# coezmaden/GPUAcceleratedTracking

Hardware: AMD Instinct MI355X
Metric: Msamples/s downconvert+correlate (E/P/L x ants x sats); real-time factor @ 1ms (higher is better)
Workload: dtype f32

## Files before the change

gpuacceleratedtracking_amd/csrc/gat_api.cpp:

```cpp
#include <algorithm>
#include <cctype>
#include <cmath>
#include <cstdio>
#include <cstdlib>
#include <cstring>
#include <ctime>
#include <dlfcn.h>
#include <new>
#include <string>
#include <vector>

#include "gat_ctx.h"

using namespace gat;

namespace gat {

struct Roctx {
    int (*push)(const char *) = nullptr;
    int (*pop)() = nullptr;
    Roctx()
    {
        const char *e = std::getenv("GAT_ROCTX");
        if (e && e[0] == '0') return;
// ... 133 lines not shown
            }
            c->loop_graphs.erase(c->loop_graphs.begin() + (long)lru);
        }
        gat_ctx::LoopGraph g;
        g.key = key;
        g.exec = exec;
        g.last_use = ++c->loop_graph_clock;
        c->loop_graphs.push_back(std::move(g));
    }
    if (graph) (void)hipGraphDestroy(graph);
    return GAT_OK;
}

void key_put_ctx(std::vector<unsigned char> &key, const gat_ctx *c)
{
    key_put(key, c->mc_mode); key_put(key, c->mc_i16_terms); key_put(key, c->mc_nct); key_put(key, c->max_aw); key_put(key, c->max_kt); key_put(key, c->max_bpw); key_put(key, c->force_bpw);
    key_put(key, c->wgs_per_cu); key_put(key, c->max_depth); key_put(key, c->one_wave); key_put(key, c->keep_l2); key_put(key, c->align_head);
    key_put(key, c->aw2); key_put(key, c->quads); key_put(key, c->bit_tables); key_put(key, c->seg_cap);
    key_put(key, c->d_codes); key_put(key, c->d_code_bits); key_put(key, c->Lc); key_put(key, c->P);
    key_put(key, c->d_partial); key_put(key, c->partial_bytes);
}

}

namespace {

struct OptionDesc {
    const char *name;
    long long lo, hi;
};
constexpr OptionDesc kOptions[] = {
// ... 3 lines not shown
    {"dc_kt", 1, 4},
    {"dc_bpw", 1, 1 << 20},
    {"dc_bpw_force", 0, 1 << 20},
    {"dc_wgs_per_cu", 0, 1024},
    {"dc_one_wave", 0, 1},
    {"dc_one_wave_min", -1, 1ll << 40},
    {"dc_ow_seg", 1, kUcarSteps},
    {"dc_depth", 1, 2},
    {"dc_keep_l2", -1, 1},
    {"dc_quads", -1, 1},
    {"dc_bits", 0, 2},
    {"dc_aw2", -1, 1},
    {"dc_seg", 0, kUcarSteps},
    {"mc_nct", 0, 4},
    {"mc_i16_terms", 2, 3},
    {"dc_align", 0, 1},
};

int32_t set_option(gat_ctx *c, const char *name, long long v)
{
    const OptionDesc *o = nullptr;
    for (const auto &d : kOptions)
        if (std::strcmp(d.name, name) == 0) o = &d;
    if (!o) return fail(c, GAT_ERR_ARG, "unknown option");
    if (v < o->lo || v > o->hi) return fail(c, GAT_ERR_RANGE, "option value out of range");
    const std::string n = name;
    if (n == "sync_flag_wgs") c->flag_max_wgs = (int)v;
    else if (n == "max_ant_tile") c->max_ant_tile = (int)v;
    else if (n == "dc_aw") c->max_aw = (int)v;
    else if (n == "dc_kt") c->max_kt = (int)v;
    else if (n == "dc_bpw") c->max_bpw = (int)v;
    else if (n == "dc_bpw_force") c->force_bpw = (int)v;
    else if (n == "dc_wgs_per_cu") c->wgs_per_cu = (int)v;
    else if (n == "dc_one_wave") c->one_wave = (int)v;
    else if (n == "dc_one_wave_min") c->one_wave_min = v;
    else if (n == "dc_ow_seg") c->one_wave_seg = (int)v;
    else if (n == "dc_depth") c->max_depth = (int)v;
    else if (n == "dc_keep_l2") c->keep_l2 = (int)v;
    else if (n == "dc_quads") c->quads = (int)v;
    else if (n == "dc_bits") c->bit_tables = (int)v;
    else if (n == "dc_aw2") c->aw2 = (int)v;
    else if (n == "dc_seg") c->seg_cap = (int)v;
    else if (n == "dc_align") c->align_head = (int)v;
    else if (n == "mc_i16_terms") c->mc_i16_terms = (int)v;
    else if (n == "mc_nct") c->mc_nct = v == 3 ? 2 : (int)v;
    return GAT_OK;
}

}

extern "C" {

GAT_API int32_t gat_create(int32_t device, void *hip_stream, gat_ctx **out_ctx)
{
    if (!out_ctx) return GAT_ERR_ARG;
    *out_ctx = nullptr;
    int ndev = 0;
    hipError_t e = hipGetDeviceCount(&ndev);
    if (e != hipSuccess) return -(int32_t)e;
// ... 621 lines not shown
```

gpuacceleratedtracking_amd/csrc/gat_ctx.h:

```cpp
#pragma once

#include <cmath>
#include <string>
#include <vector>

#include "gat_internal.h"

struct gat_ctx;

struct gat_resident {
    gat_ctx *ctx = nullptr;
    hipStream_t stream = nullptr;
    gat::DcArgs a{};
    gat::DcLaunch cfg{};
    gat::ResidentArgs r{};
    unsigned char *h_block = nullptr;
    unsigned *h_bell = nullptr, *h_state = nullptr, *h_lines = nullptr, *h_init = nullptr;
    unsigned *d_quit = nullptr;
    unsigned *d_bell = nullptr;
    int bell_copies = 1;
    int wgs = 0, lines_per_wg = 0, nval = 0;
    int blocks_per_cu = 1;
    std::vector<int> val_src, val_dst;
    unsigned seq = 0;
// ... 49 lines not shown
    int force_bpw = 0;
    int wgs_per_cu = 0;
    int one_wave = 1;
    long long one_wave_min = -1;
    int one_wave_seg = gat::kOneWaveSegSteps;
    int max_depth = 2;
    int keep_l2 = -1;
    int quads = -1;
    int bit_tables = 1;
    int aw2 = -1;
    int seg_cap = 0;
    int align_head = 1;
    int mc_mode = 1;
    int mc_nct = 0;
    int mc_i16_terms = 2;
    std::string err;
    gat_launch_info last{};
};

namespace gat {

inline int32_t fail(gat_ctx *c, int32_t code, const char *msg)
{
    if (c) c->err = msg;
    return code;
}

inline int32_t hipfail(gat_ctx *c, hipError_t e, const char *where)
{
    if (c) {
// ... 45 lines not shown
```

gpuacceleratedtracking_amd/csrc/gat_internal.h:

```cpp
#pragma once

#include <hip/hip_runtime.h>
#include <stdint.h>

#include "gat.h"

#if (defined(GAT_DC_ABLATE) || defined(GAT_DC_LAT_CUT) || defined(GAT_ABLATE) || defined(GAT_MFMA_STAMPS) || defined(GAT_MB_CW8) || defined(GAT_MB_NT_LOADS) || defined(GAT_MB_NO_RING) || defined(GAT_MB_X2_ITEMS4) || defined(GAT_MB_X2_DEPTH2) || \
     defined(GAT_RES_STAMPS) || defined(GAT_RES_FENCE)) &&                                                                                                 \
    !defined(GAT_DEV)
#error "diagnostic builds (-DGAT_DC_ABLATE, -DGAT_DC_LAT_CUT, -DGAT_ABLATE, -DGAT_MFMA_STAMPS, -DGAT_MB_CW8, -DGAT_RES_STAMPS, -DGAT_RES_FENCE) need -DGAT_DEV"
#endif

namespace gat {

constexpr int kThreads = 256;
constexpr int kMaxTapsPerLaunch = 8;
constexpr int kInlineParams = 4;
constexpr int kMaxAntTile = 4;
constexpr int kFinalizeFewSplits = 32;
constexpr int kMaxReplicaSpan = 512;
constexpr int kMaxLaunchSpan = 2048;

#ifndef GAT_PLANAR_GROUPS
#define GAT_PLANAR_GROUPS 1
// ... 205 lines not shown
constexpr int mb_consumer_waves(int, int) { return 4; }
#endif
constexpr int kMbMaxChain = 8192;
constexpr int kMbMaxSlots = 24;
constexpr int kMbHeader = 1536;
constexpr int mb_tile_samples(int RT, int NCT)
{
    const int t = 32 * (4 / NCT), cap = 128 / RT;
    return t < cap ? t : cap;
}
constexpr int mb_slots(int nct, int L, int K)
{
    const int s = (32 * nct + 2 * L - 1) / (2 * L) + 1;
    return s < K ? s : K;
}
enum MbMode : int { kMbThree = 0, kMbOne = 1, kMbTwo = 2 };
constexpr int mb_mode(int rt, int nct, int fmt, bool force_three = false)
{
    if (fmt == GAT_LAYOUT_INTERLEAVED_I8) return kMbOne;
    const int wpt = mb_consumer_waves(rt, nct) / nct, hs = mb_tile_samples(rt, nct) / (wpt > 0 ? wpt : 1) / 2;
    return fmt == GAT_LAYOUT_INTERLEAVED_I16 && !force_three && wpt > 0 && hs >= 8 && hs % 8 == 0 ? kMbTwo : kMbThree;
}
constexpr int mb_two_row_bytes(int T) { return ((10 * T + 15) / 16 * 16) | 16; }
#ifdef GAT_MB_NO_RING
constexpr bool mb_rep_ring_rows(int) { return false; }
#else
constexpr bool mb_rep_ring_rows(int rt) { return rt >= 2; }
#endif
constexpr int mb_rep_ring(int rt, int T, int span) { return mb_rep_ring_rows(rt) ? (span + 2 * T + T - 1) / T * T : 0; }
constexpr int mb_rep_row(int rt, int T, int span) { return mb_rep_ring_rows(rt) ? mb_rep_ring(rt, T, span) + span + T : span + T; }
constexpr size_t mb_lds_bytes(int rt, int nct, int fmt, int nslots, int rep_stride, int code_bits_stride, int mode = -1)
{
    if (mode < 0) mode = mb_mode(rt, nct, fmt);
    const bool x1 = mode == kMbOne;
    const int T = mb_tile_samples(rt, nct);
    const int xs = x1 ? T + 2 : T + 1, wbytes = x1 ? 8 : 16;
    const size_t xw = mode == kMbTwo ? (size_t)2 * rt * 32 * mb_two_row_bytes(T) + (size_t)2 * (2 * nslots + 1) * mb_two_row_bytes(T)
                                     : (size_t)2 * rt * 32 * xs * 8 + (size_t)2 * (2 * nslots + 1) * xs * wbytes;
    return (size_t)kMbHeader + xw + (size_t)(((mb_rep_ring_rows(rt) ? 1 : 2) * nslots * rep_stride + 3) & ~3) * 4 + (size_t)nslots * code_bits_stride * 4;
}
constexpr int kMfTile = 256;
constexpr int kMfXStride = kMfTile + 1;
constexpr size_t mf_lds_bytes(int nct, int ct, int rep_stride, int code_row_stride, int codes_in_lds)
{
    return (size_t)1024 + (size_t)2 * 32 * kMfXStride * sizeof(float) + (size_t)2 * nct * ct * rep_stride * sizeof(float) +
           (codes_in_lds ? (size_t)nct * ct * code_row_stride + 16 : 0);
}
hipError_t launch_mfma(const MfArgs &a, int nct, unsigned grid, unsigned lds_bytes, hipStream_t s);
size_t mfma_lds_bytes(int nct, int ct, int rep_stride, int code_row_stride, int codes_in_lds);
hipError_t launch_mfma_bf16(const MfArgs &a, int rt, int nct, int fmt, unsigned grid, unsigned lds_bytes, hipStream_t s);
size_t mfma_bf16_lds_bytes(int rt, int nct, int fmt, int nslots, int rep_stride, int code_bits_stride, int mode);
int mfma_bf16_mode(int rt, int nct, int fmt, bool force_three);
// ... 40 lines not shown
```

gpuacceleratedtracking_amd/csrc/gat_mfma_bf16.hip:

```cpp
#include "gat_internal.h"
#include "gat_phase.h"

#include <utility>

namespace gat {

typedef float f32x16 __attribute__((ext_vector_type(16)));
typedef float f32x4_ __attribute__((ext_vector_type(4)));
typedef short bf16x8 __attribute__((ext_vector_type(8)));
typedef unsigned u32x4 __attribute__((ext_vector_type(4)));
typedef unsigned u32x2 __attribute__((ext_vector_type(2)));

namespace {

constexpr int consumer_waves(int RT, int NCT) { return mb_consumer_waves(RT, NCT); }
constexpr int kMaxChain = kMbMaxChain;
constexpr int kReanchor = 16;
constexpr int kHeader = kMbHeader;

struct Split3 {
    unsigned v, r, r2;
};
__device__ __forceinline__ Split3 split3(float v)
{
    Split3 s;
    s.v = __float_as_uint(v);
    const float r = v - __uint_as_float(s.v & 0xffff0000u);
    s.r = __float_as_uint(r);
    s.r2 = __float_as_uint(r - __uint_as_float(s.r & 0xffff0000u));
    return s;
}
__device__ __forceinline__ void gload_nt(f32x4_ &dst, const void *p)
{
#ifdef GAT_MB_NT_LOADS
    asm volatile("global_load_dwordx4 %0, %1, off nt" : "=v"(dst) : "v"(p) : "memory");
#else
    asm volatile("global_load_dwordx4 %0, %1, off" : "=v"(dst) : "v"(p) : "memory");
#endif
}
template <int XI>
__device__ __forceinline__ void wait_loads(f32x4_ (&xv)[XI])
{
    static_assert(XI >= 1 && XI <= 4, "prefetch group size");
    if constexpr (XI == 1)
// ... 13 lines not shown
    u32x4 w;
    unsigned m;
    u32x2 xa[RT];
#if defined(GAT_ABLATE) && (GAT_ABLATE & 64)
    u32x2 wl;
#endif
};
template <int RT>
struct FragSet<RT, kMbOne> {
    u32x4 w;
    u32x2 m;
    u32x4 xa[RT];
#if defined(GAT_ABLATE) && (GAT_ABLATE & 64)
    u32x2 wl;
#endif
};
template <int RT>
struct FragSet<RT, kMbTwo> {
    u32x4 w;
    u32x2 m;
    unsigned m3;
    u32x4 xa[RT];
};
template <int RT, int XM>
constexpr int frag_reads(int J) { return XM == kMbTwo ? 2 + RT + ((J % 5 == 1 || J % 5 == 3) ? 1 : 0) : 2 + RT; }
template <int RT, int XM>
constexpr int frag_newer(int J, int n, int NM)
{
    int c = 0;
    for (int i = 1; i <= n; ++i) c += frag_reads<RT, XM>((J + i) % NM);
// ... 11 lines not shown
    }
#endif
#if defined(GAT_ABLATE) && (GAT_ABLATE & 64)
    asm volatile("ds_read_b64 %0, %1 offset:%2" : "=v"(s.wl) : "v"(w_addr), "n"(J * 16));
#else
    asm volatile("ds_read_b128 %0, %1 offset:%2" : "=v"(s.w) : "v"(w_addr), "n"(J * 16));
#endif
    if constexpr (XM == kMbTwo) {
        constexpr int j = J % 5, sb = 8 * (J / 5);
        constexpr int o0 = sb + (j == 0 ? 0 : j == 1 ? 1 : j == 2 ? 3 : j == 3 ? 4 : 6);
        asm volatile("ds_read2_b32 %0, %1 offset0:%2 offset1:%3" : "=v"(s.m) : "v"(r_addr), "n"(o0), "n"(o0 + 1));
        if constexpr (j == 1 || j == 3) asm volatile("ds_read_b32 %0, %1 offset:%2" : "=v"(s.m3) : "v"(r_addr), "n"((o0 + 2) * 4));
#pragma unroll
        for (int t = 0; t < RT; ++t)
            asm volatile("ds_read_b128 %0, %1 offset:%2" : "=v"(s.xa[t]) : "v"(x_addr[t]), "n"(J * 16));
    } else if constexpr (XM == kMbOne) {
        asm volatile("ds_read2_b32 %0, %1 offset0:%2 offset1:%3" : "=v"(s.m) : "v"(r_addr), "n"(2 * J), "n"(2 * J + 1));
#pragma unroll
        for (int t = 0; t < RT; ++t)
            asm volatile("ds_read_b128 %0, %1 offset:%2" : "=v"(s.xa[t]) : "v"(x_addr[t]), "n"(J * 16));
    } else {
        asm volatile("ds_read_b32 %0, %1 offset:%2" : "=v"(s.m) : "v"(r_addr), "n"(J * 4));
#pragma unroll
        for (int t = 0; t < RT; ++t)
            asm volatile("ds_read_b64 %0, %1 offset:%2" : "=v"(s.xa[t]) : "v"(x_addr[t]), "n"(J * 8));
    }
}
template <int RT, int XM, int NEWER>
__device__ __forceinline__ void frag_wait(FragSet<RT, XM> &s)
{
// ... 10 lines not shown
                         : "n"(NEWER));
    } else if constexpr (RT == 1)
        asm volatile("s_waitcnt lgkmcnt(%3)" : "+v"(s.w), "+v"(s.m), "+v"(s.xa[0]) : "n"(NEWER));
    else if constexpr (RT == 2)
        asm volatile("s_waitcnt lgkmcnt(%4)" : "+v"(s.w), "+v"(s.m), "+v"(s.xa[0]), "+v"(s.xa[1]) : "n"(NEWER));
    else
        asm volatile("s_waitcnt lgkmcnt(%6)"
                     : "+v"(s.w), "+v"(s.m), "+v"(s.xa[0]), "+v"(s.xa[1]), "+v"(s.xa[2]), "+v"(s.xa[3])
                     : "n"(NEWER));
}
template <int RT, int XM = kMbThree>
constexpr int frag_depth()
{
    constexpr int per = XM == kMbTwo ? 3 + RT : 2 + RT;
#ifndef GAT_MB_X2_DEPTH2
    if ((XM == kMbTwo || XM == kMbOne) && RT == 4) return 1;
#endif
    return (15 / per) < 4 ? (15 / per) : 4;
}

template <int RT, int XM>
using FragRing = FragSet<RT, XM>[frag_depth<RT, XM>() + 1];

template <int J, int RT, int XM>
__device__ __forceinline__ void mfma_apply(f32x16 (&acc)[RT == 1 ? 2 : RT], FragSet<RT, XM> &cur);

template <int J, int NM, int RT, int XM>
__device__ __forceinline__ void mfma_slice(f32x16 (&acc)[RT == 1 ? 2 : RT], FragRing<RT, XM> &fs, unsigned w_addr,
                                           unsigned r_addr, const unsigned (&x_addr)[RT])
{
    constexpr int D = frag_depth<RT, XM>();
// ... 26 lines not shown
#endif
    if constexpr (XM == kMbTwo) {
        const unsigned A = cur.m[0], B = cur.m[1], C = cur.m3;
        constexpr int j = J % 5;
        auto LH = [](unsigned a_, unsigned b_) { return GAT_PERM(b_, a_, 0x07060100u); };
        if constexpr (j == 0) { w[0] ^= A; w[1] ^= A; w[2] ^= LH(A, B); w[3] ^= B; }
        else if constexpr (j == 1) { w[0] ^= A; w[1] ^= B; w[2] ^= B; w[3] ^= LH(B, C); }
        else if constexpr (j == 2) { w[0] ^= A; w[1] ^= A; w[2] ^= B; w[3] ^= B; }
        else if constexpr (j == 3) { w[0] ^= LH(A, B); w[1] ^= B; w[2] ^= B; w[3] ^= C; }
        else { w[0] ^= A; w[1] ^= LH(A, B); w[2] ^= B; w[3] ^= B; }
        const bf16x8 bw = __builtin_bit_cast(bf16x8, w);
#pragma unroll
        for (int t = 0; t < RT; ++t)
            acc[RT == 1 ? (J & 1) : t] = __builtin_amdgcn_mfma_f32_32x32x16_bf16(__builtin_bit_cast(bf16x8, cur.xa[t]), bw,
                                                                             acc[RT == 1 ? (J & 1) : t], 0, 0, 0);
    } else if constexpr (X1) {
        const unsigned m0 = cur.m[0], m1 = cur.m[1];
        w[0] ^= m0;
        w[1] ^= m0;
        w[2] ^= m1;
        w[3] ^= m1;
        const bf16x8 bw = __builtin_bit_cast(bf16x8, w);
#pragma unroll
        for (int t = 0; t < RT; ++t)
            acc[RT == 1 ? (J & 1) : t] = __builtin_amdgcn_mfma_f32_32x32x16_bf16(__builtin_bit_cast(bf16x8, cur.xa[t]), bw,
                                                                             acc[RT == 1 ? (J & 1) : t], 0, 0, 0);
    } else {
        const unsigned mk = cur.m;
        w[0] ^= mk;
        w[1] ^= mk;
// ... 70 lines not shown
    float wTr, wTi;
    int prn, valid, bad;
    int inc_ok;
};
static_assert(sizeof(ChanInfoB) == 64, "ChanInfoB layout");

constexpr int tile_samples(int RT, int NCT) { return mb_tile_samples(RT, NCT); }

}

template <int RT, int NCT, int FMT, int XM>
__global__ void __launch_bounds__(mb_threads(RT, NCT)) mfma_bf16_kernel(const MfArgs a)
{
    static_assert((XM == kMbOne) == (FMT == GAT_LAYOUT_INTERLEAVED_I8), "one term: int8 samples, and only they");
    static_assert(XM != kMbTwo || FMT == GAT_LAYOUT_INTERLEAVED_I16, "two terms: int16 samples");
    constexpr int kMbThreads = mb_threads(RT, NCT);
    constexpr int T = tile_samples(RT, NCT);
    constexpr int NCW = consumer_waves(RT, NCT);
    constexpr int WPT = NCW / NCT;
    constexpr int SW = T / WPT;
    constexpr bool X1 = XM == kMbOne;
    constexpr bool X2 = XM == kMbTwo;
    constexpr int SPS = X1 ? 4 : 2;
    constexpr int NM = X2 ? 5 * (SW / 2) / 8 : SW / SPS;
    static_assert(!X2 || (SW / 2) % 8 == 0, "two-term stream: 8 samples per half and period");
    constexpr int OS = XM == kMbThree ? T / 2 : 1;
#ifdef GAT_MB_X2_ITEMS4
    constexpr int IS = X2 ? 4 : 2;
#else
    constexpr int IS = 2;
#endif
    constexpr int RB = mb_two_row_bytes(T);
    constexpr int XS = X1 ? T + 2 : T + 1;
    constexpr int WS = X1 ? T + 2 : T + 1;
    constexpr int WE = X1 ? 1 : 2;
    constexpr bool PLANAR = FMT == GAT_LAYOUT_PLANAR;
    constexpr int GS = PLANAR ? 4 : FMT == GAT_LAYOUT_INTERLEAVED ? 2 : FMT == GAT_LAYOUT_INTERLEAVED_I16 ? 4 : 8;
    constexpr int BYTES = FMT == GAT_LAYOUT_INTERLEAVED_I16 ? 4 : FMT == GAT_LAYOUT_INTERLEAVED_I8 ? 2 : 8;
    constexpr int QPR = T / GS;
    constexpr int PT = kMbThreads - 64 * NCW;
    constexpr int NG = (PLANAR ? RT * 32 : RT * 16) * QPR;
    extern __shared__ __attribute__((aligned(16))) unsigned char smem[];
    const int L = a.L;
    const int nslots = a.nslots;
    const int wrows = 2 * nslots + 1;
    const int RS = a.rep_stride;
    ChanInfoB *s_chan = reinterpret_cast<ChanInfoB *>(smem);
    u32x2 *s_x = reinterpret_cast<u32x2 *>(smem + kHeader);
    u32x2 *s_w = X2 ? s_x + 2 * RT * 32 * (RB / 8) : s_x + 2 * RT * 32 * XS;
    constexpr bool RINGREP = mb_rep_ring_rows(RT);
    unsigned *s_rep = reinterpret_cast<unsigned *>(X2 ? s_w + 2 * wrows * (RB / 8) : s_w + 2 * wrows * WS * WE);
    unsigned *s_code = s_rep + (((RINGREP ? 1 : 2) * nslots * RS + 3) & ~3);
    const int RR = a.rep_ring, WIN = a.rep_span + tile_samples(RT, NCT);
    auto ring_next = [RR](int s_) {
        const int n = s_ + tile_samples(RT, NCT), m = (n - RR) >> 31;
        return (n & m) | ((n - RR) & ~m);
    };

    const int tid = threadIdx.x, lane = tid & 63, wave = tid >> 6;
    const bool producer = wave >= NCW;
    const int ptid = tid - 64 * NCW;

    const unsigned xcd = blockIdx.x & 7u, jq = blockIdx.x >> 3;
    const int cg = (int)(jq % (unsigned)a.chan_groups);
    unsigned tile = (jq / (unsigned)a.chan_groups) * 8u + xcd;
    if (tile >= (unsigned)a.num_tiles) return;
// ... 19 lines not shown
            ci.phi = P.carrier_phase_cycles;
            const double sp = __builtin_fabs(ci.tau) + __builtin_fabs(ci.ratio) * (double)(N + a.max_abs_shift) + 1.0;
            ci.bad = P.prn < 0 || P.prn >= a.num_prns || !(sp < 1073741824.0) || !(sp < 2097152.0 * (double)Lc) ||
                     !(ci.ratio >= 0.0) || !(ci.ratio * 32.0 < (double)Lc) || carrier_bad(ci.step, ci.phi);
            ci.prn = (P.prn < 0 || P.prn >= a.num_prns) ? 0 : P.prn;
            if (ci.bad) { ci.ratio = 0.0; ci.tau = 0.0; ci.step = 0.0; ci.phi = 0.0; }
            carrier_reduce(ci.step, ci.phi);
            const double st_O = ci.step * (double)OS;
            sincos_cycles(st_O - __builtin_rint(st_O), ci.wr, ci.wi);
            const double st_T = ci.step * (double)T;
            sincos_cycles(st_T - __builtin_rint(st_T), ci.wTr, ci.wTi);
            ci.inc_ok = ci.ratio * (double)(T + 2) < (double)Lc;
        }
        s_chan[tid] = ci;
    }
    if constexpr (X2) {
        for (int e = tid; e < 2 * (RB / 8); e += kMbThreads)
            s_w[((e / (RB / 8)) * wrows + 2 * nslots) * (RB / 8) + e % (RB / 8)] = u32x2{0u, 0u};
    } else {
        for (int e = tid; e < 2 * WS * WE; e += kMbThreads)
            s_w[((e / (WS * WE)) * wrows * WS + 2 * nslots * WS) * WE + e % (WS * WE)] = u32x2{0u, 0u};
    }
    __syncthreads();
    {
        const int vec_per_row = a.code_bits_stride / 4;
        for (int e = tid; e < nslots * vec_per_row; e += kMbThreads) {
            const int slot = e / vec_per_row, v = e - slot * vec_per_row;
            const ChanInfoB c = s_chan[slot];
            if (c.valid)
                reinterpret_cast<uint4 *>(s_code)[slot * vec_per_row + v] =
                    reinterpret_cast<const uint4 *>(a.code_bits + (size_t)c.prn * a.code_bits_stride)[v];
// ... 68 lines not shown
                    u32x2 *d = reinterpret_cast<u32x2 *>(reinterpret_cast<unsigned char *>(xb) + plane * RB + 40 * q);
                    d[0] = u32x2{GAT_P2(A[0], A[0]), GAT_P2(B[0], A[0])};
                    d[1] = u32x2{GAT_P2(A[1], B[0]), GAT_P2(A[1], A[1])};
                    d[2] = u32x2{GAT_P2(B[1], B[1]), GAT_P2(A[2], A[2])};
                    d[3] = u32x2{GAT_P2(B[2], A[2]), GAT_P2(A[3], B[2])};
                    d[4] = u32x2{GAT_P2(A[3], A[3]), GAT_P2(B[3], B[3])};
                };
                put4(2 * row, ar, br);
                put4(2 * row + 1, ai, bi);
                continue;
            }
            auto put = [&](int plane, int rel, float v) {
                if constexpr (X1) {
                    const unsigned fb = __float_as_uint(v);
                    xb[plane * XS + rel] = u32x2{GAT_PERM(fb, fb, 0x03020302u), fb >> 16};
                } else {
#if defined(GAT_ABLATE) && (GAT_ABLATE & 128)
                    const unsigned fb = __float_as_uint(v);
                    const float r = v - __uint_as_float(fb & 0xffff0000u);
                    xb[plane * XS + rel] = u32x2{GAT_PERM(__float_as_uint(r), fb, 0x07060302u), 0u};
#else
                    const Split3 sp = split3(v);
                    xb[plane * XS + rel] = u32x2{GAT_PERM(sp.r, sp.v, 0x07060302u), GAT_PERM(sp.r2, sp.r2, 0x03020302u)};
#endif
                }
            };
            if constexpr (PLANAR) {
#pragma unroll
                for (int u = 0; u < 4; ++u) put(row, 4 * q + u, xv[it][u]);
            } else if constexpr (FMT == GAT_LAYOUT_INTERLEAVED) {
// ... 47 lines not shown
                row[e] = m;
                return;
            }
            int q = win + e;
            q -= q >= RR ? RR : 0;
            row[q] = m;
            if (q < WIN) row[RR + q] = m;
        };
        put(e0, m0);
        if (e0 + dist < e_end) put(e0 + dist, m1);
    };
    float car_r = 0.f, car_i = 0.f;
    int rep_ip = 0, rep_t = 0, rep_ip2 = 0, rep_t2 = 0;
    const int item_i = ptid / (T / IS), item_q = ptid % (T / IS);
    const int item_slot = X2 ? ((item_i & ~3) | ((item_i & 1) << 1) | ((item_i >> 1) & 1)) : item_i;
    const int item_s0 = X2 ? IS * item_q : X1 ? 2 * item_q : item_q;
    const bool have_item = producer && item_slot < nslots;
    int p_win = 0;
    auto produce = [&](int st, int buf, bool first) {
        const int nb = st * T;
        const int win = p_win;
        if constexpr (RINGREP) p_win = ring_next(p_win);
        u32x2 *wb = X2 ? s_w + buf * wrows * (RB / 8) : s_w + buf * wrows * WS * WE;
        unsigned *rb = RINGREP ? s_rep : s_rep + buf * nslots * RS;
        const ChanInfoB c = s_chan[have_item ? item_slot : 0];
        if (first) {
            const int gps = (span + 1) >> 1;
            for (int id = ptid; id < nslots * gps; id += PT) {
                const int slot = id / gps, g = id - slot * gps;
                const ChanInfoB cs = s_chan[slot];
                if (!cs.valid) continue;
                int ip_unused, t_unused;
                gen_rep2(cs, s_code + slot * a.code_bits_stride, rb + slot * RS, win, nb, 2 * g, 1, span, true, ip_unused, t_unused);
            }
        } else if constexpr (!RINGREP) {
            const unsigned *rprev = s_rep + (buf ^ 1) * nslots * RS;
            const int pw = wave - NCW;
            for (int slot = pw; slot < nslots; slot += PT / 64)
// ... 13 lines not shown
                         anchor || !c.inc_ok, rep_ip2, rep_t2);
        }
#if defined(GAT_ABLATE) && (GAT_ABLATE & 2)
        if (!first) return;
#endif
        float cr, ci;
        if (anchor) {
            const double th = __builtin_fma((double)(nb + item_s0), c.step, c.phi);
            sincos_cycles(th - __builtin_rint(th), cr, ci);
        } else {
            cr = __builtin_fmaf(car_r, c.wTr, -(car_i * c.wTi));
            ci = __builtin_fmaf(car_r, c.wTi, car_i * c.wTr);
        }
        car_r = cr;
        car_i = ci;
        if constexpr (X2 && IS == 2) {
            const Split3 c0 = split3(cr), s0 = split3(-ci);
            const float tr = __builtin_fmaf(cr, c.wr, -(ci * c.wi));
            ci = __builtin_fmaf(cr, c.wi, ci * c.wr);
            cr = tr;
            const Split3 c1 = split3(cr), s1 = split3(-ci);
            unsigned *dre = reinterpret_cast<unsigned *>(reinterpret_cast<unsigned char *>(wb) + (2 * item_slot) * RB + 20 * item_q);
            unsigned *dim = reinterpret_cast<unsigned *>(reinterpret_cast<unsigned char *>(dre) + RB);
            dre[0] = GAT_P2(c0.r, c0.v); dre[1] = GAT_P2(c0.v, c0.r2); dre[2] = GAT_P2(c1.v, c0.r); dre[3] = GAT_P2(c1.r2, c1.r); dre[4] = GAT_P2(c1.r, c1.v);
            dim[0] = GAT_P2(s0.r, s0.v); dim[1] = GAT_P2(s0.v, s0.r2); dim[2] = GAT_P2(s1.v, s0.r); dim[3] = GAT_P2(s1.r2, s1.r); dim[4] = GAT_P2(s1.r, s1.v);
            return;
        } else if constexpr (X2) {
            unsigned ch[4], cm[4], cl[4], sh[4], sm[4], sl[4];
#pragma unroll
            for (int u = 0; u < 4; ++u) {
                const Split3 sc = split3(cr), ss = split3(-ci);
// ... 41 lines not shown
        }
    };

    const int cw = producer ? 0 : wave;
    const int ctl = cw / WPT;
    const int sub = cw % WPT;
    const int r = lane & 31, h = lane >> 5;
    const int col = 32 * (NCT * cg + ctl) + r;
    const int k_col = col / (2 * L), rem_col = col - 2 * L * k_col;
    const int l = rem_col >> 1, comp = rem_col & 1;
    const bool in_range = k_col < a.K && k_col - k_first < nslots;
    const int slot_c = in_range ? k_col - k_first : 0;
    const ChanInfoB my = s_chan[slot_c];
    const bool live_col = in_range && my.valid;
    const int col0 = sub * SW + h * (SW / 2);
    const int w_off = X2 ? (live_col ? 2 * slot_c + comp : 2 * nslots) * RB + 10 * col0 : (live_col ? 2 * slot_c + comp : 2 * nslots) * WS + col0;
    const int r_off = slot_c * RS + (a.shifts[l] - a.shifts[0]) + col0;
    const int x_off = X2 ? r * RB + 10 * col0 : r * XS + col0;
    constexpr int XBUF = X2 ? RT * 32 * RB : 8 * RT * 32 * XS, XTILE = X2 ? 32 * RB : 8 * 32 * XS, XU = X2 ? 1 : 8;
    const int WBUF = X2 ? wrows * RB : 8 * WE * wrows * WS, WU = X2 ? 1 : 8 * WE;

    if (!producer) __builtin_amdgcn_s_setprio(3);

    constexpr int NA = RT == 1 ? 2 : RT;
    f32x16 acc[NA];
#pragma unroll
    for (int t = 0; t < NA; ++t)
#pragma unroll
        for (int i = 0; i < 16; ++i) acc[t][i] = 0.f;

    const unsigned lds_x = (unsigned)(uintptr_t)s_x, lds_w = (unsigned)(uintptr_t)s_w, lds_r = (unsigned)(uintptr_t)s_rep;
    int c_win = 0;
    auto consume = [&](int buf) {
#if defined(GAT_ABLATE) && (GAT_ABLATE & 8)
        return;
// ... 212 lines not shown

int mfma_bf16_slots(int nct, int L, int K) { return mb_slots(nct, L, K); }

size_t mfma_bf16_lds_bytes(int rt, int nct, int fmt, int nslots, int rep_stride, int code_bits_stride, int mode)
{
    static_assert(sizeof(ChanInfoB) * kMbMaxSlots <= kHeader, "channel table must fit the header");
    return mb_lds_bytes(rt, nct, fmt, nslots, rep_stride, code_bits_stride, mode);
}
int mfma_bf16_mode(int rt, int nct, int fmt, bool force_three) { return mb_mode(rt, nct, fmt, force_three); }

namespace {
template <int RT, int NCT, int F>
hipError_t launch_one(const MfArgs &a, dim3 g, dim3 blk, unsigned lds_bytes, hipStream_t s)
{
    constexpr int natural = F == GAT_LAYOUT_INTERLEAVED_I8 ? kMbOne : kMbThree;
    if constexpr (mb_mode(RT, NCT, F) == kMbTwo) {
        if (a.mb_mode == kMbTwo) {
            hipLaunchKernelGGL((mfma_bf16_kernel<RT, NCT, F, kMbTwo>), g, blk, lds_bytes, s, a);
            return hipSuccess;
        }
    }
    if (a.mb_mode != natural) return hipErrorInvalidValue;
    hipLaunchKernelGGL((mfma_bf16_kernel<RT, NCT, F, natural>), g, blk, lds_bytes, s, a);
    return hipSuccess;
}
}

hipError_t launch_mfma_bf16(const MfArgs &a, int rt, int nct, int fmt, unsigned grid, unsigned lds_bytes, hipStream_t s)
{
    const dim3 g(grid), blk(mb_threads(rt, nct));
// ... 20 lines not shown
```

gpuacceleratedtracking_amd/csrc/gat_planner.cpp:

```cpp
#include <algorithm>
#include <cctype>
#include <cmath>
#include <cstdio>
#include <cstdlib>
#include <cstring>
#include <ctime>
#include <dlfcn.h>
#include <new>
#include <string>
#include <vector>

#include "gat_ctx.h"

using namespace gat;

int32_t gat::correlate_impl(gat_ctx *c, const gat_signal_desc *sig, const gat_channel_params *params_dev,
                            int32_t B, int32_t K, int32_t L, const int32_t *shifts, double fs,
                            float *out_re, float *out_im, uint32_t flags, const gat_channel_params *params_inline,
                            DcPlan *plan_out)
{
    c->wait_seq = 0;
    const TraceRange trace("gat_downconvert_and_correlate");
    if (!sig || (!params_dev && !params_inline) || !shifts || !out_re || !out_im) return fail(c, GAT_ERR_ARG, "null argument");
    if (!c->d_codes) return fail(c, GAT_ERR_STATE, "gat_set_codes has not been called");
// ... 90 lines not shown
        const bool round2_rule = M >= 32 && K >= 32 && (long long)M * K >= 2048;
        const bool auto_bf16 = 2ll * L * K >= 24 && (int8_in || (L <= 3 ? util >= util_min : round2_rule));
        const bool auto_f32 = false;
        const bool want_bf16 = c->mc_mode == 3 || (c->mc_mode == 1 && auto_bf16);
        const bool want_f32 = c->mc_mode == 2 || (c->mc_mode == 1 && auto_f32);
        int kind = 0, rt = 1, rep_stride_m = 0;
        int nslots_b = 0, nct_b = 1;
        if (shape_any && want_bf16 && c->d_code_bits && c->d_zeros && N % spv == 0 && spv <= 8) {
            if (c->mc_nct > 0) n_first = c->mc_nct;
            for (int n = n_first; n >= 1 && !kind; n >>= 1) {
                rt = (rt_max == 4 && n == 1) ? 2 : rt_max;
                const int T = mfma_bf16_tile_samples(rt, n);
                int rs = ((mb_rep_row(rt, T, (int)span) + 31) / 32) * 32 + 1;
                const int ns = mfma_bf16_slots(n, L, K);
                if (ns * T / 2 > mfma_bf16_producer_threads(rt, n) || ns > mfma_bf16_max_slots()) continue;
                const int mode_n = mfma_bf16_mode(rt, n, fmt, c->mc_i16_terms == 3);
                const int rs_tuned = pick_rep_stride(rs - 1, tiles_b, order);
                if (mfma_bf16_lds_bytes(rt, n, fmt, ns, rs_tuned, c->code_bits_stride, mode_n) <= 160 * 1024) rs = rs_tuned;
                if (mfma_bf16_lds_bytes(rt, n, fmt, ns, rs, c->code_bits_stride, mode_n) <= 160 * 1024) {
                    if (c->mc_mode == 1) {
                        const long long steps_total = (N + T - 1) / T;
                        const long long groups = (long long)B * (M / (16 * rt)) * ((tiles_b + n - 1) / n);
                        const long long cut = std::min<long long>(steps_total, std::max<long long>(1, (2ll * c->num_cus + groups - 1) / groups));
                        const long long steps_each = (steps_total + cut - 1) / cut;
                        if (steps_each < (two_term || int8_in ? 16 : 32)) break;
                    }
                    kind = 2;
                    nct_b = n;
                    nslots_b = ns;
                    rep_stride_m = rs;
                }
// ... 76 lines not shown
            m.partial = c->d_partial;
#ifdef GAT_MFMA_STAMPS
            {
                static unsigned long long *dbg = nullptr;
                if (!dbg) hipMalloc(reinterpret_cast<void **>(&dbg), 8u << 20);
                m.dbg = dbg;
                c->dbg_ptr = dbg;
            }
#endif
            unsigned lds;
            if (kind == 2) {
                m.codes_in_lds = 1;
                m.code_bits = c->d_code_bits;
                m.zeros = c->d_zeros;
                m.code_bits_stride = c->code_bits_stride;
                m.mb_mode = mfma_bf16_mode(rt, nct, fmt, c->mc_i16_terms == 3);
                lds = (unsigned)mfma_bf16_lds_bytes(rt, nct, fmt, m.nslots, m.rep_stride, c->code_bits_stride, m.mb_mode);
                GAT_HIP(c, launch_mfma_bf16(m, rt, nct, fmt, (unsigned)grid_m, lds, c->stream));
            } else {
                m.codes_in_lds = mfma_lds_bytes(nct, CT, m.rep_stride, c->code_row_stride, 1) <= 160 * 1024;
                lds = (unsigned)mfma_lds_bytes(nct, CT, m.rep_stride, c->code_row_stride, m.codes_in_lds);
                GAT_HIP(c, launch_mfma(m, nct, (unsigned)grid_m, lds, c->stream));
            }
            const bool fin_m = !atomic_m && m.splits > 1;
            if (fin_m)
                GAT_HIP(c, launch_finalize(c->d_partial, out_re, out_im, m.splits, L * M * 2, (long long)B * K, c->stream));
            c->last.workgroups = (int32_t)grid_m;
            c->last.threads = kind == 2 ? mfma_bf16_threads(rt, nct) : 2 * kThreads;
            c->last.splits = m.splits;
            c->last.ant_tile = kind == 2 ? 16 * rt : 16;
            c->last.vec = 4;
// ... 274 lines not shown
```

Measured before the change: 214,500.

## Add six-product bf16 split mode for float samples in MFMA correlator

Adds a kMbSix mode for f32 planar/interleaved samples. Each sample and carrier value is split into three RNE bf16 terms, and only six of the nine cross products are fed to the MFMA, replacing the previous three-term path. It packs the carrier terms into 12-byte-per-sample rows and reads them with ds_read2/ds_read_b128 patterns. The aim is to cut MFMA and LDS work per sample while keeping near-f32 accuracy, at the risk of slight precision loss and extra producer split work. It is on by default (mc_f32_products=6) and can be turned off via an option.

```diff
diff --git a/gpuacceleratedtracking_amd/csrc/gat_api.cpp b/gpuacceleratedtracking_amd/csrc/gat_api.cpp
--- a/gpuacceleratedtracking_amd/csrc/gat_api.cpp
+++ b/gpuacceleratedtracking_amd/csrc/gat_api.cpp
@@ -171,7 +171,7 @@
 
 void key_put_ctx(std::vector<unsigned char> &key, const gat_ctx *c)
 {
-    key_put(key, c->mc_mode); key_put(key, c->mc_i16_terms); key_put(key, c->mc_nct); key_put(key, c->max_aw); key_put(key, c->max_kt); key_put(key, c->max_bpw); key_put(key, c->force_bpw);
+    key_put(key, c->mc_mode); key_put(key, c->mc_i16_terms); key_put(key, c->mc_f32_products); key_put(key, c->mc_nct); key_put(key, c->max_aw); key_put(key, c->max_kt); key_put(key, c->max_bpw); key_put(key, c->force_bpw);
     key_put(key, c->wgs_per_cu); key_put(key, c->max_depth); key_put(key, c->one_wave); key_put(key, c->keep_l2); key_put(key, c->align_head);
     key_put(key, c->aw2); key_put(key, c->quads); key_put(key, c->bit_tables); key_put(key, c->seg_cap);
     key_put(key, c->d_codes); key_put(key, c->d_code_bits); key_put(key, c->Lc); key_put(key, c->P);
@@ -205,6 +205,7 @@
     {"dc_seg", 0, kUcarSteps},
     {"mc_nct", 0, 4},
     {"mc_i16_terms", 2, 3},
+    {"mc_f32_products", 6, 8},
     {"dc_align", 0, 1},
 };
 
@@ -215,6 +216,7 @@
         if (std::strcmp(d.name, name) == 0) o = &d;
     if (!o) return fail(c, GAT_ERR_ARG, "unknown option");
     if (v < o->lo || v > o->hi) return fail(c, GAT_ERR_RANGE, "option value out of range");
+    if (std::strcmp(name, "mc_f32_products") == 0 && v == 7) return fail(c, GAT_ERR_RANGE, "option value out of range");
     const std::string n = name;
     if (n == "sync_flag_wgs") c->flag_max_wgs = (int)v;
     else if (n == "max_ant_tile") c->max_ant_tile = (int)v;
@@ -234,6 +236,7 @@
     else if (n == "dc_seg") c->seg_cap = (int)v;
     else if (n == "dc_align") c->align_head = (int)v;
     else if (n == "mc_i16_terms") c->mc_i16_terms = (int)v;
+    else if (n == "mc_f32_products") c->mc_f32_products = (int)v;
     else if (n == "mc_nct") c->mc_nct = v == 3 ? 2 : (int)v;
     return GAT_OK;
 }
diff --git a/gpuacceleratedtracking_amd/csrc/gat_ctx.h b/gpuacceleratedtracking_amd/csrc/gat_ctx.h
--- a/gpuacceleratedtracking_amd/csrc/gat_ctx.h
+++ b/gpuacceleratedtracking_amd/csrc/gat_ctx.h
@@ -87,6 +87,7 @@
     int mc_mode = 1;
     int mc_nct = 0;
     int mc_i16_terms = 2;
+    int mc_f32_products = 6;
     std::string err;
     gat_launch_info last{};
 };
diff --git a/gpuacceleratedtracking_amd/csrc/gat_internal.h b/gpuacceleratedtracking_amd/csrc/gat_internal.h
--- a/gpuacceleratedtracking_amd/csrc/gat_internal.h
+++ b/gpuacceleratedtracking_amd/csrc/gat_internal.h
@@ -243,14 +243,17 @@
     const int s = (32 * nct + 2 * L - 1) / (2 * L) + 1;
     return s < K ? s : K;
 }
-enum MbMode : int { kMbThree = 0, kMbOne = 1, kMbTwo = 2 };
-constexpr int mb_mode(int rt, int nct, int fmt, bool force_three = false)
+enum MbMode : int { kMbThree = 0, kMbOne = 1, kMbTwo = 2, kMbSix = 3 };
+constexpr int mb_mode(int rt, int nct, int fmt, bool force_three = false, int f32_products = 6)
 {
     if (fmt == GAT_LAYOUT_INTERLEAVED_I8) return kMbOne;
     const int wpt = mb_consumer_waves(rt, nct) / nct, hs = mb_tile_samples(rt, nct) / (wpt > 0 ? wpt : 1) / 2;
+    if (fmt == GAT_LAYOUT_PLANAR || fmt == GAT_LAYOUT_INTERLEAVED)
+        return f32_products == 6 && wpt > 0 && hs >= 4 && hs % 4 == 0 ? kMbSix : kMbThree;
     return fmt == GAT_LAYOUT_INTERLEAVED_I16 && !force_three && wpt > 0 && hs >= 8 && hs % 8 == 0 ? kMbTwo : kMbThree;
 }
 constexpr int mb_two_row_bytes(int T) { return ((10 * T + 15) / 16 * 16) | 16; }
+constexpr int mb_six_row_bytes(int T) { return ((12 * T + 15) / 16 * 16) | 16; }
 #ifdef GAT_MB_NO_RING
 constexpr bool mb_rep_ring_rows(int) { return false; }
 #else
@@ -261,10 +264,11 @@
 constexpr size_t mb_lds_bytes(int rt, int nct, int fmt, int nslots, int rep_stride, int code_bits_stride, int mode = -1)
 {
     if (mode < 0) mode = mb_mode(rt, nct, fmt);
-    const bool x1 = mode == kMbOne;
+    const bool x1 = mode == kMbOne, x6 = mode == kMbSix;
     const int T = mb_tile_samples(rt, nct);
-    const int xs = x1 ? T + 2 : T + 1, wbytes = x1 ? 8 : 16;
+    const int xs = x1 || x6 ? T + 2 : T + 1, wbytes = x1 ? 8 : 16;
     const size_t xw = mode == kMbTwo ? (size_t)2 * rt * 32 * mb_two_row_bytes(T) + (size_t)2 * (2 * nslots + 1) * mb_two_row_bytes(T)
+                      : x6           ? (size_t)2 * rt * 32 * xs * 8 + (size_t)2 * (2 * nslots + 1) * mb_six_row_bytes(T)
                                      : (size_t)2 * rt * 32 * xs * 8 + (size_t)2 * (2 * nslots + 1) * xs * wbytes;
     return (size_t)kMbHeader + xw + (size_t)(((mb_rep_ring_rows(rt) ? 1 : 2) * nslots * rep_stride + 3) & ~3) * 4 + (size_t)nslots * code_bits_stride * 4;
 }
diff --git a/gpuacceleratedtracking_amd/csrc/gat_mfma_bf16.hip b/gpuacceleratedtracking_amd/csrc/gat_mfma_bf16.hip
--- a/gpuacceleratedtracking_amd/csrc/gat_mfma_bf16.hip
+++ b/gpuacceleratedtracking_amd/csrc/gat_mfma_bf16.hip
@@ -28,6 +28,17 @@
     const float r = v - __uint_as_float(s.v & 0xffff0000u);
     s.r = __float_as_uint(r);
     s.r2 = __float_as_uint(r - __uint_as_float(s.r & 0xffff0000u));
+    return s;
+}
+__device__ __forceinline__ unsigned bf16_rne(unsigned u) { return (u + 0x7fffu + ((u >> 16) & 1u)) & 0xffff0000u; }
+__device__ __forceinline__ Split3 split3_rne(float v)
+{
+    Split3 s;
+    const float big = __uint_as_float(0x7f7f0000u);
+    s.v = bf16_rne(__float_as_uint(__builtin_amdgcn_fmed3f(v, -big, big)));
+    const float r = v - __uint_as_float(s.v);
+    s.r = bf16_rne(__float_as_uint(r));
+    s.r2 = __float_as_uint(r - __uint_as_float(s.r));
     return s;
 }
 __device__ __forceinline__ void gload_nt(f32x4_ &dst, const void *p)
@@ -71,6 +82,12 @@
 #if defined(GAT_ABLATE) && (GAT_ABLATE & 64)
     u32x2 wl;
 #endif
+};
+template <int RT>
+struct FragSet<RT, kMbSix> {
+    u32x4 w;
+    u32x2 m;
+    u32x4 xa[RT];
 };
 template <int RT>
 struct FragSet<RT, kMbTwo> {
@@ -112,6 +129,16 @@
 #pragma unroll
         for (int t = 0; t < RT; ++t)
             asm volatile("ds_read_b128 %0, %1 offset:%2" : "=v"(s.xa[t]) : "v"(x_addr[t]), "n"(J * 16));
+    } else if constexpr (XM == kMbSix) {
+        constexpr int j = J % 3, sb = 4 * (J / 3);
+        asm volatile("ds_read2_b32 %0, %1 offset0:%2 offset1:%3" : "=v"(s.m) : "v"(r_addr), "n"(sb + j), "n"(sb + j + 1));
+#pragma unroll
+        for (int t = 0; t < RT; ++t) {
+            if constexpr (j == 1)
+                asm volatile("ds_read2_b64 %0, %1 offset0:%2 offset1:%3" : "=v"(s.xa[t]) : "v"(x_addr[t]), "n"(sb + 1), "n"(sb + 2));
+            else
+                asm volatile("ds_read_b128 %0, %1 offset:%2" : "=v"(s.xa[t]) : "v"(x_addr[t]), "n"(8 * (sb + j)));
+        }
     } else if constexpr (XM == kMbOne) {
         asm volatile("ds_read2_b32 %0, %1 offset0:%2 offset1:%3" : "=v"(s.m) : "v"(r_addr), "n"(2 * J), "n"(2 * J + 1));
 #pragma unroll
@@ -152,7 +179,8 @@
 {
     constexpr int per = XM == kMbTwo ? 3 + RT : 2 + RT;
 #ifndef GAT_MB_X2_DEPTH2
-    if ((XM == kMbTwo || XM == kMbOne) && RT == 4) return 1;
+    if ((XM == kMbTwo || XM == kMbOne || XM == kMbSix) && RT == 4) return 1;
+    if (XM == kMbSix && RT == 2) return 2;
 #endif
     return (15 / per) < 4 ? (15 / per) : 4;
 }
@@ -209,6 +237,20 @@
         for (int t = 0; t < RT; ++t)
             acc[RT == 1 ? (J & 1) : t] = __builtin_amdgcn_mfma_f32_32x32x16_bf16(__builtin_bit_cast(bf16x8, cur.xa[t]), bw,
                                                                              acc[RT == 1 ? (J & 1) : t], 0, 0, 0);
+    } else if constexpr (XM == kMbSix) {
+        const unsigned A = cur.m[0], B = cur.m[1];
+        constexpr int j = J % 3;
+        if constexpr (j == 0) { w[0] ^= A; w[1] ^= A; w[2] ^= A; w[3] ^= B; }
+        else if constexpr (j == 1) { w[0] ^= A; w[1] ^= A; w[2] ^= B; w[3] ^= B; }
+        else { w[0] ^= A; w[1] ^= B; w[2] ^= B; w[3] ^= B; }
+        const bf16x8 bw = __builtin_bit_cast(bf16x8, w);
+#pragma unroll
+        for (int t = 0; t < RT; ++t) {
+            const u32x4 v = cur.xa[t];
+            const u32x4 xf = j == 0 ? u32x4{v[0], v[0], v[1], v[2]} : j == 1 ? u32x4{v[0], v[1], v[2], v[2]} : u32x4{v[1], v[2], v[2], v[3]};
+            acc[RT == 1 ? (J & 1) : t] = __builtin_amdgcn_mfma_f32_32x32x16_bf16(__builtin_bit_cast(bf16x8, xf), bw,
+                                                                             acc[RT == 1 ? (J & 1) : t], 0, 0, 0);
+        }
     } else if constexpr (X1) {
         const unsigned m0 = cur.m[0], m1 = cur.m[1];
         w[0] ^= m0;
@@ -309,6 +351,7 @@
 {
     static_assert((XM == kMbOne) == (FMT == GAT_LAYOUT_INTERLEAVED_I8), "one term: int8 samples, and only they");
     static_assert(XM != kMbTwo || FMT == GAT_LAYOUT_INTERLEAVED_I16, "two terms: int16 samples");
+    static_assert(XM != kMbSix || FMT == GAT_LAYOUT_PLANAR || FMT == GAT_LAYOUT_INTERLEAVED, "six products: float samples");
     constexpr int kMbThreads = mb_threads(RT, NCT);
     constexpr int T = tile_samples(RT, NCT);
     constexpr int NCW = consumer_waves(RT, NCT);
@@ -316,17 +359,20 @@
     constexpr int SW = T / WPT;
     constexpr bool X1 = XM == kMbOne;
     constexpr bool X2 = XM == kMbTwo;
+    constexpr bool X6 = XM == kMbSix;
     constexpr int SPS = X1 ? 4 : 2;
-    constexpr int NM = X2 ? 5 * (SW / 2) / 8 : SW / SPS;
+    constexpr int NM = X2 ? 5 * (SW / 2) / 8 : X6 ? 3 * (SW / 2) / 4 : SW / SPS;
     static_assert(!X2 || (SW / 2) % 8 == 0, "two-term stream: 8 samples per half and period");
+    static_assert(!X6 || (SW / 2) % 4 == 0, "six-product stream: 4 samples per half and period");
     constexpr int OS = XM == kMbThree ? T / 2 : 1;
 #ifdef GAT_MB_X2_ITEMS4
     constexpr int IS = X2 ? 4 : 2;
 #else
     constexpr int IS = 2;
 #endif
-    constexpr int RB = mb_two_row_bytes(T);
-    constexpr int XS = X1 ? T + 2 : T + 1;
+    constexpr int RB = X6 ? mb_six_row_bytes(T) : mb_two_row_bytes(T);
+    constexpr bool WROW = X2 || X6;
+    constexpr int XS = X1 || X6 ? T + 2 : T + 1;
     constexpr int WS = X1 ? T + 2 : T + 1;
     constexpr int WE = X1 ? 1 : 2;
     constexpr bool PLANAR = FMT == GAT_LAYOUT_PLANAR;
@@ -344,7 +390,7 @@
     u32x2 *s_x = reinterpret_cast<u32x2 *>(smem + kHeader);
     u32x2 *s_w = X2 ? s_x + 2 * RT * 32 * (RB / 8) : s_x + 2 * RT * 32 * XS;
     constexpr bool RINGREP = mb_rep_ring_rows(RT);
-    unsigned *s_rep = reinterpret_cast<unsigned *>(X2 ? s_w + 2 * wrows * (RB / 8) : s_w + 2 * wrows * WS * WE);
+    unsigned *s_rep = reinterpret_cast<unsigned *>(WROW ? s_w + 2 * wrows * (RB / 8) : s_w + 2 * wrows * WS * WE);
     unsigned *s_code = s_rep + (((RINGREP ? 1 : 2) * nslots * RS + 3) & ~3);
     const int RR = a.rep_ring, WIN = a.rep_span + tile_samples(RT, NCT);
     auto ring_next = [RR](int s_) {
@@ -394,7 +440,7 @@
         }
         s_chan[tid] = ci;
     }
-    if constexpr (X2) {
+    if constexpr (WROW) {
         for (int e = tid; e < 2 * (RB / 8); e += kMbThreads)
             s_w[((e / (RB / 8)) * wrows + 2 * nslots) * (RB / 8) + e % (RB / 8)] = u32x2{0u, 0u};
     } else {
@@ -493,6 +539,9 @@
                 if constexpr (X1) {
                     const unsigned fb = __float_as_uint(v);
                     xb[plane * XS + rel] = u32x2{GAT_PERM(fb, fb, 0x03020302u), fb >> 16};
+                } else if constexpr (X6) {
+                    const Split3 sp = split3_rne(v);
+                    xb[plane * XS + rel] = u32x2{GAT_P2(sp.r, sp.v), GAT_P2(sp.r2, sp.v)};
                 } else {
 #if defined(GAT_ABLATE) && (GAT_ABLATE & 128)
                     const unsigned fb = __float_as_uint(v);
@@ -570,14 +619,14 @@
     int rep_ip = 0, rep_t = 0, rep_ip2 = 0, rep_t2 = 0;
     const int item_i = ptid / (T / IS), item_q = ptid % (T / IS);
     const int item_slot = X2 ? ((item_i & ~3) | ((item_i & 1) << 1) | ((item_i >> 1) & 1)) : item_i;
-    const int item_s0 = X2 ? IS * item_q : X1 ? 2 * item_q : item_q;
+    const int item_s0 = X2 ? IS * item_q : X1 || X6 ? 2 * item_q : item_q;
     const bool have_item = producer && item_slot < nslots;
     int p_win = 0;
     auto produce = [&](int st, int buf, bool first) {
         const int nb = st * T;
         const int win = p_win;
         if constexpr (RINGREP) p_win = ring_next(p_win);
-        u32x2 *wb = X2 ? s_w + buf * wrows * (RB / 8) : s_w + buf * wrows * WS * WE;
+        u32x2 *wb = WROW ? s_w + buf * wrows * (RB / 8) : s_w + buf * wrows * WS * WE;
         unsigned *rb = RINGREP ? s_rep : s_rep + buf * nslots * RS;
         const ChanInfoB c = s_chan[have_item ? item_slot : 0];
         if (first) {
@@ -621,7 +670,22 @@
         }
         car_r = cr;
         car_i = ci;
-        if constexpr (X2 && IS == 2) {
+        if constexpr (X6) {
+            const Split3 c0 = split3_rne(cr), s0 = split3_rne(-ci);
+            const float tr = __builtin_fmaf(cr, c.wr, -(ci * c.wi));
+            ci = __builtin_fmaf(cr, c.wi, ci * c.wr);
+            cr = tr;
+            const Split3 c1 = split3_rne(cr), s1 = split3_rne(-ci);
+            u32x2 *dre = reinterpret_cast<u32x2 *>(reinterpret_cast<unsigned char *>(wb) + (2 * item_slot) * RB + 24 * item_q);
+            u32x2 *dim = reinterpret_cast<u32x2 *>(reinterpret_cast<unsigned char *>(dre) + RB);
+            dre[0] = u32x2{GAT_P2(c0.v, c0.v), GAT_P2(c0.r, c0.r)};
+            dre[1] = u32x2{GAT_P2(c0.v, c0.r2), GAT_P2(c1.v, c1.v)};
+            dre[2] = u32x2{GAT_P2(c1.r, c1.r), GAT_P2(c1.v, c1.r2)};
+            dim[0] = u32x2{GAT_P2(s0.v, s0.v), GAT_P2(s0.r, s0.r)};
+            dim[1] = u32x2{GAT_P2(s0.v, s0.r2), GAT_P2(s1.v, s1.v)};
+            dim[2] = u32x2{GAT_P2(s1.r, s1.r), GAT_P2(s1.v, s1.r2)};
+            return;
+        } else if constexpr (X2 && IS == 2) {
             const Split3 c0 = split3(cr), s0 = split3(-ci);
             const float tr = __builtin_fmaf(cr, c.wr, -(ci * c.wi));
             ci = __builtin_fmaf(cr, c.wi, ci * c.wr);
@@ -693,11 +757,12 @@
     const ChanInfoB my = s_chan[slot_c];
     const bool live_col = in_range && my.valid;
     const int col0 = sub * SW + h * (SW / 2);
-    const int w_off = X2 ? (live_col ? 2 * slot_c + comp : 2 * nslots) * RB + 10 * col0 : (live_col ? 2 * slot_c + comp : 2 * nslots) * WS + col0;
+    const int w_off = WROW ? (live_col ? 2 * slot_c + comp : 2 * nslots) * RB + (X6 ? 12 : 10) * col0
+                           : (live_col ? 2 * slot_c + comp : 2 * nslots) * WS + col0;
     const int r_off = slot_c * RS + (a.shifts[l] - a.shifts[0]) + col0;
     const int x_off = X2 ? r * RB + 10 * col0 : r * XS + col0;
     constexpr int XBUF = X2 ? RT * 32 * RB : 8 * RT * 32 * XS, XTILE = X2 ? 32 * RB : 8 * 32 * XS, XU = X2 ? 1 : 8;
-    const int WBUF = X2 ? wrows * RB : 8 * WE * wrows * WS, WU = X2 ? 1 : 8 * WE;
+    const int WBUF = WROW ? wrows * RB : 8 * WE * wrows * WS, WU = WROW ? 1 : 8 * WE;
 
     if (!producer) __builtin_amdgcn_s_setprio(3);
 
@@ -940,6 +1005,12 @@
 hipError_t launch_one(const MfArgs &a, dim3 g, dim3 blk, unsigned lds_bytes, hipStream_t s)
 {
     constexpr int natural = F == GAT_LAYOUT_INTERLEAVED_I8 ? kMbOne : kMbThree;
+    if constexpr (mb_mode(RT, NCT, F) == kMbSix) {
+        if (a.mb_mode == kMbSix) {
+            hipLaunchKernelGGL((mfma_bf16_kernel<RT, NCT, F, kMbSix>), g, blk, lds_bytes, s, a);
+            return hipSuccess;
+        }
+    }
     if constexpr (mb_mode(RT, NCT, F) == kMbTwo) {
         if (a.mb_mode == kMbTwo) {
             hipLaunchKernelGGL((mfma_bf16_kernel<RT, NCT, F, kMbTwo>), g, blk, lds_bytes, s, a);
diff --git a/gpuacceleratedtracking_amd/csrc/gat_planner.cpp b/gpuacceleratedtracking_amd/csrc/gat_planner.cpp
--- a/gpuacceleratedtracking_amd/csrc/gat_planner.cpp
+++ b/gpuacceleratedtracking_amd/csrc/gat_planner.cpp
@@ -128,7 +128,7 @@
                 int rs = ((mb_rep_row(rt, T, (int)span) + 31) / 32) * 32 + 1;
                 const int ns = mfma_bf16_slots(n, L, K);
                 if (ns * T / 2 > mfma_bf16_producer_threads(rt, n) || ns > mfma_bf16_max_slots()) continue;
-                const int mode_n = mfma_bf16_mode(rt, n, fmt, c->mc_i16_terms == 3);
+                const int mode_n = mb_mode(rt, n, fmt, c->mc_i16_terms == 3, c->mc_f32_products);
                 const int rs_tuned = pick_rep_stride(rs - 1, tiles_b, order);
                 if (mfma_bf16_lds_bytes(rt, n, fmt, ns, rs_tuned, c->code_bits_stride, mode_n) <= 160 * 1024) rs = rs_tuned;
                 if (mfma_bf16_lds_bytes(rt, n, fmt, ns, rs, c->code_bits_stride, mode_n) <= 160 * 1024) {
@@ -235,7 +235,7 @@
                 m.code_bits = c->d_code_bits;
                 m.zeros = c->d_zeros;
                 m.code_bits_stride = c->code_bits_stride;
-                m.mb_mode = mfma_bf16_mode(rt, nct, fmt, c->mc_i16_terms == 3);
+                m.mb_mode = mb_mode(rt, nct, fmt, c->mc_i16_terms == 3, c->mc_f32_products);
                 lds = (unsigned)mfma_bf16_lds_bytes(rt, nct, fmt, m.nslots, m.rep_stride, c->code_bits_stride, m.mb_mode);
                 GAT_HIP(c, launch_mfma_bf16(m, rt, nct, fmt, (unsigned)grid_m, lds, c->stream));
             } else {
```

After: 213,000, median of 6. No clear change (-0.7%).
